# Jaybro/pico_tree

Measured on AMD Instinct MI355X. Metric: Mqueries/sec, knn=1 3D L2, 7.73M-pt tree / 7.20M queries, higher is better.
Workload: dtype f32; 1 GPU; BASELINE configs[1]: cloud L (LiDAR-like room scan), 7733372 tree points / 7200863 queries, knn=1, max_leaf_size=10, sliding midpoint; query_order=generated, reorder=auto, streams=1, parallelism=one batch of 7200863 queries cut into 1 shards, tree replicated, tree_nodes=2395585, tree_depth=32

## Files before the change

### pico_tree_amd/build.py

```python

from __future__ import annotations

import os
import shlex
import subprocess
import sys
from concurrent.futures import ThreadPoolExecutor

_HERE = os.path.dirname(os.path.abspath(__file__))
ROOT = os.path.dirname(_HERE)
CSRC = os.path.join(_HERE, "csrc")
LIB = os.path.join(CSRC, "libptk.so")
OBJ = os.path.join(CSRC, "_obj")
UNITS = ["ptk_family_knn", "ptk_backend", "ptk_family_nd", "ptk_family_radius", "ptk_family_f64", "ptk_family_self",
         "ptk_family_topo", "ptk_family_count"]
SOURCES = [os.path.join(CSRC, u + ".hip") for u in UNITS]

FLAGS = [
    "--offload-arch=gfx950",
    "-O3",
    "-std=c++17",
    "-ffp-contract=off",
    "-fPIC",
    "-Wall",
    "-Wno-unused-result",
    "-Wno-unused-function",
]


def _compile_flags() -> list:
    return FLAGS + os.environ.get("PTK_EXTRA_FLAGS", "").split() + [
        "-I" + os.path.join(ROOT, "include"),
        "-I" + CSRC,
    ]


def _deps(depfile: str) -> list:
    try:
        with open(depfile) as f:
            text = f.read()
    except OSError:
        return []
    text = text.replace("\\\n", " ")
    _, _, rest = text.partition(":")
    return shlex.split(rest)


def _signature(unit: str, flags_line: str) -> str:
    import hashlib

    h = hashlib.sha256(flags_line.replace(os.path.realpath(ROOT), "<root>").replace(ROOT, "<root>").encode())
    deps = sorted(set(os.path.realpath(p) for p in _deps(os.path.join(OBJ, unit + ".d"))))
    root = os.path.realpath(ROOT) + os.sep
    mine = [p for p in deps if p.startswith(root)]
    if not mine:
        return ""
    for p in mine:
        try:
            with open(p, "rb") as f:
                h.update(p[len(root):].encode() + b"\0" + f.read())
        except OSError:
            return ""
    return h.hexdigest()


def _unit_stale(unit: str, flags_line: str) -> bool:
    obj = os.path.join(OBJ, unit + ".o")
    sigfile = os.path.join(OBJ, unit + ".sig")
    if not (os.path.exists(obj) and os.path.exists(sigfile)):
        return True
    with open(sigfile) as f:
        recorded = f.read().strip()
    return recorded == "" or recorded != _signature(unit, flags_line)


def _compile(unit: str, flags: list, flags_line: str, verbose: bool) -> None:
    hipcc = os.environ.get("HIPCC", "/opt/rocm/bin/hipcc")
    obj = os.path.join(OBJ, unit + ".o")
    cmd = [hipcc] + flags + ["-c", "-MD", "-MF", os.path.join(OBJ, unit + ".d"), "-o", obj,
                             os.path.join(CSRC, unit + ".hip")]
    if verbose:
        print(" ".join(cmd), file=sys.stderr)
    subprocess.check_call(cmd)
    with open(os.path.join(OBJ, unit + ".sig"), "w") as f:
        f.write(_signature(unit, flags_line))


def build(force: bool = False, verbose: bool = False, lib: str = LIB) -> str:
    flags = _compile_flags()
    flags_line = " ".join(flags)
    os.makedirs(OBJ, exist_ok=True)
    todo = [u for u in UNITS if force or _unit_stale(u, flags_line)]
    if todo:
        jobs = max(1, min(len(todo), int(os.environ.get("PTK_BUILD_JOBS", os.cpu_count() or 4))))
        with ThreadPoolExecutor(max_workers=jobs) as pool:
            for _ in pool.map(lambda u: _compile(u, flags, flags_line, verbose), todo):
                pass
    objs = [os.path.join(OBJ, u + ".o") for u in UNITS]
    linked = os.path.join(OBJ, os.path.basename(lib) + ".sig")
    want = "\n".join(open(os.path.join(OBJ, u + ".sig")).read() for u in UNITS)
    have = open(linked).read() if os.path.exists(linked) else None
    if todo or not os.path.exists(lib) or have != want:
        hipcc = os.environ.get("HIPCC", "/opt/rocm/bin/hipcc")
        cmd = [hipcc, "--offload-arch=gfx950", "-shared", "-fPIC", "-o", lib] + objs
        if verbose:
            print(" ".join(cmd), file=sys.stderr)
        subprocess.check_call(cmd)
        with open(linked, "w") as f:
            f.write(want)
    return lib


if __name__ == "__main__":
    print(build(force="--force" in sys.argv, verbose=True))
```

### pico_tree_amd/csrc/ptk_backend.hip

```cpp

#include "ptk_families.hpp"
#include "ptk_kernels_lists.hpp"
#include "ptk_piles.hpp"
#include "ptk_build.hpp"
#include "ptk_sort.hpp"
#include "ptk_forest.hpp"
#include "ptk_rows_out.hpp"

namespace {

void axis_bits(const ptk_tree* t, int bits, uint32_t b[3]);

struct CreateClock {
  bool on;
  double* sink;
  std::chrono::steady_clock::time_point t0;
  explicit CreateClock(double* phases = nullptr)
      : on(env_int("PTK_CREATE_TIMING", 0) != 0), sink(phases), t0(std::chrono::steady_clock::now()) {}
  void lap(const char* what, int slot) {
    const auto t1 = std::chrono::steady_clock::now();
    const double ms = std::chrono::duration<double, std::milli>(t1 - t0).count();
    if (sink != nullptr && slot >= 0) sink[slot] += ms;
    if (on) std::fprintf(stderr, "[ptk create] %-28s %8.2f ms\n", what, ms);
    t0 = t1;
// ... 225 lines not shown
  std::mutex lock;
  std::thread threads[kMaxDevices];
  bool started[kMaxDevices] = {};
  void start(int32_t device) {
    if (device == kDeviceNone) return;
    const char* sw = std::getenv("PTK_EAGER_WARMUP");
    if (sw != nullptr && std::atoi(sw) == 0) return;
    int dev = device;
    if (dev < 0 && hipGetDevice(&dev) != hipSuccess) return;
    if (dev < 0 || dev >= kMaxDevices) return;
    std::lock_guard<std::mutex> hold(lock);
    if (started[dev]) return;
    started[dev] = true;
    threads[dev] = std::thread([dev] {
      if (hipSetDevice(dev) != hipSuccess) {
        (void)hipGetLastError();
        return;
      }
      hipLaunchKernelGGL(ptk_warm_kernel, dim3(1), dim3(1), 0, nullptr);
      ptkf::warm_knn();
      ptkf::warm_radius();
      ptkf::warm_nd();
      ptkf::warm_topo();
      ptkf::warm_count();
      ptkf::warm_f64();
      ptkf::warm_self();
      (void)hipDeviceSynchronize();
      (void)hipGetLastError();
    });
  }
  void wait(int32_t device) {
    int dev = device;
    if (dev < 0 && hipGetDevice(&dev) != hipSuccess) return;
    if (dev < 0 || dev >= kMaxDevices) return;
    std::lock_guard<std::mutex> hold(lock);
    if (threads[dev].joinable()) threads[dev].join();
  }
  ~ProcessWarmup() {
    for (auto& th : threads)
      if (th.joinable()) th.join();
  }
};
ProcessWarmup g_warmup;

int finish_create(ptk_tree* t, const float* points, int32_t device, ptk_tree** out) {
  if (t->root_min.empty()) {
    t->root_min.assign(t->dim, std::numeric_limits<float>::max());
    t->root_max.assign(t->dim, std::numeric_limits<float>::lowest());
    for (uint64_t i = 0; i < t->n_points; ++i)
      for (uint32_t d = 0; d < t->dim; ++d) {
        const float v = points[i * t->dim + d];
        t->root_min[d] = std::min(t->root_min[d], v);
        t->root_max[d] = std::max(t->root_max[d], v);
      }
  }
  if (device == kDeviceNone) {
    int rc = analyse(*t);
    if (rc != PTK_OK) {
      delete t;
      return rc;
    }
    t->device = kDeviceNone;
    *out = t;
    return PTK_OK;
  }
  int count = 0;
  if (hipGetDeviceCount(&count) != hipSuccess || count <= 0) {
    delete t;
    return fail(PTK_ERR_DEVICE, "no HIP device is visible");
  }
  int dev = device;
  if (dev < 0 && hipGetDevice(&dev) != hipSuccess) dev = 0;
  if (dev >= count) {
    delete t;
    return fail(PTK_ERR_INVALID, "device %d out of range (%d visible)", dev, count);
  }
  t->device = dev;
  DeviceGuard guard(dev);
  if (!guard.ok) {
    delete t;
    return fail(PTK_ERR_DEVICE, "hipSetDevice(%d) failed", dev);
  }
  {
    hipDeviceProp_t prop;
    if (hipGetDeviceProperties(&prop, dev) == hipSuccess) {
      if (prop.multiProcessorCount > 0) t->cus = prop.multiProcessorCount;
      if (prop.maxSharedMemoryPerMultiProcessor > 0) t->lds_per_cu = prop.maxSharedMemoryPerMultiProcessor;
      const size_t optin = prop.sharedMemPerBlockOptin > 0 ? (size_t)prop.sharedMemPerBlockOptin : (size_t)prop.sharedMemPerBlock;
      if (optin > 0) t->lds_per_block = std::min(optin, t->lds_per_cu);
      t->hbm_bytes = prop.totalGlobalMem;
    } else {
      (void)hipGetLastError();
    }
  }
  int rc = upload(*t, points);
  if (rc != PTK_OK) {
    ptk_tree_destroy(t);
    return rc;
  }
  *out = t;
  return PTK_OK;
}

bool want_reorder(const ptk_tree* t, uint64_t nq) {
  const int mode = t->reorder.load();
  if (mode == PTK_REORDER_ON) return nq > 1;
  if (mode == PTK_REORDER_OFF) return false;
  return nq >= 8192;
}

int morton_bits(uint64_t nq) { return nq < (1ull << 20) ? 16 : 24; }

void axis_bits(const ptk_tree* t, int bits, uint32_t b[3]) {
  b[0] = b[1] = b[2] = 0;
  const uint32_t axes = t->dim < 3 ? t->dim : 3;
  double want[3] = {0, 0, 0};
  const double total = t->axis_splits[0] + t->axis_splits[1] + t->axis_splits[2];
  for (uint32_t a = 0; a < axes; ++a) want[a] = total > 0.0 ? bits * t->axis_splits[a] / total : (double)bits / axes;
  for (int given = 0; given < bits; ++given) {
    int best = -1;
    for (uint32_t a = 0; a < axes; ++a)
      if (b[a] < 15 && (best < 0 || want[a] - b[a] > want[best] - b[best])) best = (int)a;
    if (best < 0) break;
    ++b[best];
  }
}

using MortonSortConfig =
    rocprim::radix_sort_config<rocprim::default_config, rocprim::default_config, rocprim::default_config, 131072>;

size_t sort_tmp_bytes(uint64_t nq, int bits) {
  size_t tmp_bytes = 0;
  uint32_t* k32 = nullptr;
  (void)rocprim::radix_sort_pairs<MortonSortConfig>(nullptr, tmp_bytes, k32, k32, k32, k32, nq, 0, bits,
                                                    (hipStream_t) nullptr);
  return tmp_bytes + 256;
}

uint32_t sort_tile(uint64_t nq) {
  const uint64_t t = ((nq + 4095) / 4096 + 63) & ~(uint64_t)63;
  return (uint32_t)std::max<uint64_t>(t, (uint64_t)512);
}
uint32_t sort_tiles(uint64_t nq) { return (uint32_t)((nq + sort_tile(nq) - 1) / sort_tile(nq)); }
uint32_t sort_stride(uint64_t nq) { return (sort_tiles(nq) + 3u) & ~3u;  }
size_t own_sort_bytes(uint64_t nq) {
  const size_t stride = std::max<size_t>(sort_stride(nq), ((nq + ptk::kSortTile - 1) / ptk::kSortTile + 3) & ~(size_t)3);
  return ((size_t)ptk::kRadixBins * stride + ptk::kRadixBins) * 4 + 2 * nq * sizeof(uint2) + 1024;
}

bool block_sort(uint64_t nq) {
  const int mode = knob_int("sort_block", -1);
  return mode < 0 ? nq >= (3ull << 18) : mode != 0 && nq >= ptk::kSortTile;
}
bool own_sort(uint64_t nq) {
  if (nq >= (1ull << 31)) return false;
  return knob_int("sort", 1) != 0;
}

size_t permutation_scratch_bytes(uint64_t nq) { return 4 * (nq * 4) + sort_tmp_bytes(nq, 30) + own_sort_bytes(nq) + 1024; }

const uint32_t* sample_batch(const ptk_tree* t, const float* d_q, uint64_t nq, hipStream_t s, Scratch& scratch, int bits,
                             const float3& lo3, const float3& inv3, const uint3& b3) {
  if (nq < 8192) return nullptr;
  uint8_t* d_fail = scratch.take<uint8_t>(ptk::kCoherenceWindows);
  uint32_t* state = scratch.sample_state();
  if (d_fail == nullptr || state == nullptr) return nullptr;
  uint32_t lg = 0;
  while ((128ull << lg) <= nq) ++lg;
  const uint32_t max_log2 = (uint32_t)std::min(bits, std::max(bits - (int)lg, 0) + 5);
  hipLaunchKernelGGL(ptk::coherence_sample_kernel, dim3(ptk::kCoherenceWindows), dim3(64), 0, s, d_q, t->dim, nq, lo3, inv3,
                     b3, max_log2, d_fail, state);
  return state + 1;
}

int make_permutation(const ptk_tree* t, const float* d_q, uint64_t nq, hipStream_t s, Scratch& scratch,
                     uint32_t** perm, uint32_t heavy_first = 0, bool may_skip = false) {
  *perm = nullptr;
  if (nq >= (1ull << 32)) return fail(PTK_ERR_UNSUPPORTED, "batches of 2^32 or more queries are not supported");
  Timer timer(t, s);
  const int bits = morton_bits(nq);
  size_t tmp_bytes = sort_tmp_bytes(nq, bits);
  uint32_t* keys = scratch.take<uint32_t>(nq);
  uint32_t* keys_out = scratch.take<uint32_t>(nq);
  uint32_t* ids = scratch.take<uint32_t>(nq);
  uint32_t* ids_out = scratch.take<uint32_t>(nq);
  void* tmp = scratch.take<char>(tmp_bytes);
  if (!keys || !keys_out || !ids || !ids_out || !tmp) return fail(PTK_ERR_NOMEM, "scratch block too small");
  uint32_t b[3];
  axis_bits(t, bits, b);
  float lo[3] = {0, 0, 0}, inv[3] = {0, 0, 0};
  for (uint32_t d = 0; d < t->dim && d < 3; ++d) {
    lo[d] = t->root_min[d];
    const float ext = t->root_max[d] - t->root_min[d];
    inv[d] = ext > 0 ? (float)(1u << b[d]) / ext : 0.0f;
  }
  ptk::CellTable cells{};
  if (heavy_first != 0u && t->cells.occ != nullptr) {
    cells = t->cells;
    cells.key_bits = (uint32_t)bits;
    cells.mode = heavy_first;
  }
  const uint32_t* as_given = may_skip && own_sort(nq)
                                 ? sample_batch(t, d_q, nq, s, scratch, bits, make_float3(lo[0], lo[1], lo[2]),
                                                make_float3(inv[0], inv[1], inv[2]), make_uint3(b[0], b[1], b[2]))
                                 : nullptr;
  scratch.note_verdict(as_given);
  if (own_sort(nq)) {
    const bool blocks = block_sort(nq);
    const uint32_t tile = blocks ? ptk::kSortTile : sort_tile(nq);
    const uint32_t tiles = blocks ? (uint32_t)((nq + tile - 1) / tile) : sort_tiles(nq);
    const uint32_t stride = blocks ? (tiles + 3u) & ~3u : sort_stride(nq);
    uint32_t* hist = scratch.take<uint32_t>((size_t)ptk::kRadixBins * stride);
    uint32_t* totals = scratch.take<uint32_t>(ptk::kRadixBins);
    uint2* pairs_a = scratch.take<uint2>(nq);
    uint2* pairs_b = bits > 16 ? scratch.take<uint2>(nq) : pairs_a;
    if (!hist || !totals || !pairs_a || !pairs_b) return fail(PTK_ERR_NOMEM, "scratch block too small");
    const float3 lo3 = make_float3(lo[0], lo[1], lo[2]), inv3 = make_float3(inv[0], inv[1], inv[2]);
    const uint3 b3 = make_uint3(b[0], b[1], b[2]);
    const int passes = (bits + 7) / 8;
    const size_t smem = ptk::kRadixBins * 4;
    const uint2* in = nullptr;
    for (int p = 0; p < passes; ++p) {
      const uint32_t shift = 8u * (uint32_t)p;
      const bool first = p == 0, last = p + 1 == passes;
      uint2* out = in == pairs_a ? pairs_b : pairs_a;
      if (blocks && first)
        hipLaunchKernelGGL((ptk::radix_block_hist_kernel<true>), dim3(tiles), dim3(ptk::kSortBlock), smem, s, d_q, t->dim,
                           (uint32_t)nq, lo3, inv3, b3, keys, in, shift, stride, hist, cells, as_given);
      else if (blocks)
        hipLaunchKernelGGL((ptk::radix_block_hist_kernel<false>), dim3(tiles), dim3(ptk::kSortBlock), smem, s, d_q, t->dim,
                           (uint32_t)nq, lo3, inv3, b3, keys, in, shift, stride, hist, ptk::CellTable{}, as_given);
      else if (first)
        hipLaunchKernelGGL((ptk::radix_hist_kernel<true>), dim3(tiles), dim3(64), smem, s, d_q, t->dim, (uint32_t)nq, lo3,
                           inv3, b3, keys, in, shift, tile, stride, hist, cells, as_given);
      else
        hipLaunchKernelGGL((ptk::radix_hist_kernel<false>), dim3(tiles), dim3(64), smem, s, d_q, t->dim, (uint32_t)nq, lo3,
                           inv3, b3, keys, in, shift, tile, stride, hist, ptk::CellTable{}, as_given);
      hipLaunchKernelGGL(ptk::radix_scan_kernel, dim3(ptk::kRadixBins), dim3(64), 0, s, hist, tiles, stride, totals);
#define PTK_SCATTER(F, L)                                                                                              \
  if (blocks)                                                                                                          \
    hipLaunchKernelGGL((ptk::radix_block_scatter_kernel<F, L>), dim3(tiles), dim3(ptk::kSortBlock),                    \
                       ptk::kSortScatterLds, s, keys, in, out, ids_out, (uint32_t)nq, shift, stride, hist, totals,     \
                       as_given);                                                                                      \
  else                                                                                                                 \
    hipLaunchKernelGGL((ptk::radix_scatter_kernel<F, L>), dim3(tiles), dim3(64), smem, s, keys, in, out, ids_out,      \
                       (uint32_t)nq, shift, tile, stride, hist, totals, as_given)
      if (first && last) PTK_SCATTER(true, true);
      else if (first) PTK_SCATTER(true, false);
      else if (last) PTK_SCATTER(false, true);
      else PTK_SCATTER(false, false);
#undef PTK_SCATTER
      in = out;
    }
    PTK_HIP(hipGetLastError());
    *perm = ids_out;
    scratch.note_order(1);
    timer.stop(1, 0);
    return PTK_OK;
  }
  {
    const uint32_t blocks = (uint32_t)((nq + ptk::kBlock - 1) / ptk::kBlock);
    hipLaunchKernelGGL(ptk::morton_kernel, dim3(blocks), dim3(ptk::kBlock), 0, s, d_q, t->dim, nq,
                       make_float3(lo[0], lo[1], lo[2]), make_float3(inv[0], inv[1], inv[2]),
                       make_uint3(b[0], b[1], b[2]), keys, ids, cells, (uint64_t)0);
  }
  PTK_HIP(rocprim::radix_sort_pairs<MortonSortConfig>(tmp, tmp_bytes, keys, keys_out, ids, ids_out, nq, 0, bits, s));
  *perm = ids_out;
  scratch.note_order(1);
  timer.stop(1, 0);
  return PTK_OK;
}

int order_batch(const ptk_tree* t, const float* d_q, uint64_t nq, hipStream_t s, Scratch& scratch, size_t extra_bytes,
                uint32_t** perm, uint32_t heavy_first = 0, bool may_skip = false) {
  *perm = nullptr;
  const bool reorder = want_reorder(t, nq);
  const int rc = scratch.reserve(extra_bytes + (reorder ? permutation_scratch_bytes(nq) : 0));
  if (rc != PTK_OK || !reorder) return rc;
  return make_permutation(t, d_q, nq, s, scratch, perm, heavy_first, may_skip);
}

size_t capture_budget_bytes(const ptk_tree* t) {
  const size_t quarter_mb = t->hbm_bytes ? (t->hbm_bytes >> 22) : 16384;
  const int mb = env_int("PTK_RADIUS_CAPTURE_MB", (int)std::min<size_t>(16384, std::max<size_t>(quarter_mb, 64)));
  return mb <= 0 ? 0 : (size_t)mb << 20;
}

bool prepare_capture(const ptk_tree* t, uint64_t nq, Workspace& ws, bool with_heavy = false) {
  const size_t budget = capture_budget_bytes(t);
  if (budget == 0 || nq == 0 || nq >= (1ull << 31)) return false;
  const size_t waves = (size_t)((nq + 63) / 64);
  const size_t chunk_bytes = (size_t)ptk::kLogChunk * sizeof(ptk::Neighbor);
  const size_t flags_at = (size_t)ptk::kCapSubPools * ptk::kCapCounterStride * 4;
  const size_t qids_at = flags_at + ((waves + 255) & ~(size_t)255);
  const size_t lens_at = qids_at + waves * 64 * 4;
  const size_t tables_at = lens_at + waves * 64 * 4;
  const size_t heavy_at = (tables_at + waves * ptk::kListMaxChunks * 4 + 255) & ~(size_t)255;
  const size_t mh = with_heavy ? (size_t)radius_max_handover(nq) : 0, ecap = with_heavy ? (size_t)radius_entry_cap(nq) : 0;
  const size_t heavy_bytes = with_heavy ? 256 + 4 * ((mh * 4 + 255) & ~(size_t)255) + ecap * 8 : 0;
  const size_t head = (heavy_at + heavy_bytes + 4095) & ~(size_t)4095;
  if (head + waves * chunk_bytes > budget) return false;
  const size_t dyn = std::min<size_t>((budget - head - waves * chunk_bytes) / chunk_bytes, waves * 64 * 2);
  const int forced = knob_int("radius_capture_chunks", -1);
  size_t sub_cap = forced >= 0 ? (size_t)forced : dyn / ptk::kCapSubPools;
  const size_t max_chunks = ((1ull << 32) - 1) / ptk::kLogChunk;
  if (waves >= max_chunks) return false;
  if (waves + sub_cap * ptk::kCapSubPools > max_chunks) sub_cap = (max_chunks - waves) / ptk::kCapSubPools;
  const size_t bytes = head + (waves + sub_cap * ptk::kCapSubPools) * chunk_bytes;
  if (bytes > ws.cap_capacity) {
    drain_workspace(ws);
    if (ws.cap_base) (void)hipFree(ws.cap_base);
    ws.cap_base = nullptr;
    ws.cap_capacity = 0;
    ws.cap_valid = false;
    size_t free_b = 0, total_b = 0;
    if (hipMemGetInfo(&free_b, &total_b) != hipSuccess || bytes > free_b / 2) return false;
    if (hipMalloc((void**)&ws.cap_base, bytes) != hipSuccess) {
      (void)hipGetLastError();
      ws.cap_base = nullptr;
      return false;
    }
    ws.cap_capacity = bytes;
  }
  ws.cap.counters = reinterpret_cast<uint32_t*>(ws.cap_base);
  ws.cap.captured = reinterpret_cast<uint8_t*>(ws.cap_base + flags_at);
  ws.cap.qids = reinterpret_cast<uint32_t*>(ws.cap_base + qids_at);
  ws.cap.lens = reinterpret_cast<uint32_t*>(ws.cap_base + lens_at);
  ws.cap.tables = reinterpret_cast<uint32_t*>(ws.cap_base + tables_at);
  ws.cap.chunks = reinterpret_cast<ptk::Neighbor*>(ws.cap_base + head);
  ws.cap.n_static = (uint32_t)waves;
  ws.cap.sub_cap = (uint32_t)sub_cap;
  ws.cap_heavy = ptk::RadiusHeavy{};
  if (with_heavy) {
    const size_t row = (mh * 4 + 255) & ~(size_t)255;
    char* p = ws.cap_base + heavy_at;
    ws.cap_heavy.meta = reinterpret_cast<uint32_t*>(p);
    ws.cap_heavy.rows = reinterpret_cast<uint32_t*>(p + 256);
    ws.cap_heavy.own = reinterpret_cast<uint32_t*>(p + 256 + row);
    ws.cap_heavy.run_at = reinterpret_cast<uint32_t*>(p + 256 + 2 * row);
    ws.cap_heavy.run_n = reinterpret_cast<uint32_t*>(p + 256 + 3 * row);
    ws.cap_heavy.entries = reinterpret_cast<unsigned long long*>(p + 256 + 4 * row);
    ws.cap_heavy.max_heavy = (uint32_t)mh;
    ws.cap_heavy.entry_cap = (uint32_t)std::min<size_t>(ecap, 0xFFFFFFFFu);
  }
  return true;
}

ptk::TierSpec phase2_tiers(uint32_t cap) {
  ptk::TierSpec t{};
  if (cap == 0) {
    t.permille[0] = 60;
    t.lanes[0] = 4;
  }
  return t;
}

size_t class_sort_tmp_bytes(uint64_t nq) {
  size_t tmp_bytes = 0;
  ptk::ContKey* k16 = nullptr;
  uint32_t* v32 = nullptr;
  (void)rocprim::radix_sort_pairs(nullptr, tmp_bytes, k16, k16, v32, v32, nq, 0, 16, (hipStream_t) nullptr);
  return tmp_bytes + 256;
}

uint64_t max_handover(uint64_t nq) { return std::max<uint64_t>(nq / 32, std::min<uint64_t>(nq, 16384)); }

struct ClassPlan {
  uint32_t ntiles, stride, seg, segs, per, chunks;
};
ClassPlan class_plan(uint64_t nq) {
  ClassPlan p;
  p.ntiles = (uint32_t)((nq + 63) / 64);
  p.stride = (p.ntiles + 3u) & ~3u;
// ... 2099 lines not shown
```

### pico_tree_amd/csrc/ptk_sort.hpp

```cpp

#pragma once

#include <hip/hip_runtime.h>
#include <stdint.h>

#include "ptk_kernels.hpp"

namespace ptk {

constexpr uint32_t kRadixBins = 256;

__device__ __forceinline__ uint64_t same_digit_lanes(uint32_t digit, bool valid) {
  uint64_t peers = __ballot(valid);
#pragma unroll
  for (uint32_t b = 0; b < 8; ++b) {
    const bool bit = ((digit >> b) & 1u) != 0u;
    const uint64_t m = __ballot(bit);
    peers &= bit ? m : ~m;
  }
  return peers;
}

__device__ __forceinline__ uint32_t wave_inclusive_sum(uint32_t v, uint32_t lane) {
#pragma unroll
// ... 148 lines not shown
        const uint32_t dst = p + (uint32_t)__popcll(peers & below);
        if (LAST) vals_out[dst] = val[u];
        else pairs_out[dst] = make_uint2(key[u], val[u]);
        if ((peers >> lane) == 1ull) pos[digit] = p + (uint32_t)__popcll(peers);
      }
    }
  }
}

constexpr uint32_t kSortBlock = 512, kSortItems = 8, kSortTile = kSortBlock * kSortItems;
constexpr uint32_t sort_scatter_lds(uint32_t block, uint32_t items) {
  return ((block / 64u) * kRadixBins + 2u * kRadixBins + 32u) * 4u + block * items * 8u;
}
constexpr uint32_t kSortScatterLds = sort_scatter_lds(kSortBlock, kSortItems);

__device__ __forceinline__ uint32_t block_exclusive_sum(uint32_t v, uint32_t t, PTK_LDS uint32_t* tmp) {
  const uint32_t lane = t & 63u, w = t >> 6;
  const uint32_t incl = wave_inclusive_sum(v, lane);
  if (lane == 63u && w < 4u) tmp[w] = incl;
  __syncthreads();
  uint32_t before = 0;
#pragma unroll
  for (uint32_t j = 0; j < 3; ++j) before += j < w ? tmp[j] : 0u;
  __syncthreads();
  return before + incl - v;
}

template <bool FROM_QUERIES, uint32_t BLOCK = kSortBlock, uint32_t ITEMS = kSortItems>
__global__ __launch_bounds__(BLOCK) void radix_block_hist_kernel(
    const float* __restrict__ queries, uint32_t dim, uint32_t nq, float3 lo, float3 inv, uint3 bits,
    uint32_t* __restrict__ keys, const uint2* __restrict__ pairs, uint32_t shift, uint32_t stride,
    uint32_t* __restrict__ hist, CellTable cells = CellTable{}, const uint32_t* __restrict__ as_given = nullptr) {
  if (as_given != nullptr && *as_given != 0u) return;
  typedef PTK_LDS uint32_t LdsU32;
  LdsU32* cnt = (LdsU32*)ptk_smem;
  const uint32_t t = threadIdx.x;
  if (t < kRadixBins) cnt[t] = 0u;
  __syncthreads();
  const uint32_t base = blockIdx.x * (BLOCK * ITEMS);
  uint32_t key[ITEMS];
  bool valid[ITEMS];
  if (FROM_QUERIES) {
    float x[ITEMS], y[ITEMS], z[ITEMS];
#pragma unroll
    for (uint32_t j = 0; j < ITEMS; ++j) {
      const uint32_t i = base + j * BLOCK + t;
      valid[j] = i < nq;
      load_query(queries, dim, valid[j] ? i : nq - 1u, x[j], y[j], z[j]);
    }
#pragma unroll
    for (uint32_t j = 0; j < ITEMS; ++j) {
      key[j] = order_key(x[j], y[j], z[j], lo, inv, bits, cells);
      if (valid[j]) keys[base + j * BLOCK + t] = key[j];
    }
  } else {
#pragma unroll
    for (uint32_t j = 0; j < ITEMS; ++j) {
      const uint32_t i = base + j * BLOCK + t;
      valid[j] = i < nq;
      key[j] = valid[j] ? pairs[i].x : 0u;
    }
  }
#pragma unroll
  for (uint32_t j = 0; j < ITEMS; ++j) {
    if (valid[j]) lds_add_u32(&cnt[(key[j] >> shift) & 255u], 1u);
  }
  __syncthreads();
  if (t < kRadixBins) hist[t * stride + blockIdx.x] = cnt[t];
}

template <bool FIRST, bool LAST, uint32_t BLOCK = kSortBlock, uint32_t ITEMS = kSortItems>
__global__ __launch_bounds__(BLOCK) void radix_block_scatter_kernel(
    const uint32_t* __restrict__ keys_in, const uint2* __restrict__ pairs_in, uint2* __restrict__ pairs_out,
    uint32_t* __restrict__ vals_out, uint32_t n, uint32_t shift, uint32_t stride, const uint32_t* __restrict__ hist,
    const uint32_t* __restrict__ totals, const uint32_t* __restrict__ as_given = nullptr) {
  if (as_given != nullptr && *as_given != 0u) return;
  constexpr uint32_t WAVES = BLOCK / 64u, TILE = BLOCK * ITEMS;
  static_assert(BLOCK >= kRadixBins && BLOCK % 64u == 0u, "a thread per digit");
  typedef PTK_LDS uint32_t LdsU32;
  LdsU32* wave_cnt = (LdsU32*)ptk_smem;
  LdsU32* lbase = wave_cnt + WAVES * kRadixBins;
  LdsU32* gbase = lbase + kRadixBins;
  LdsU32* tmp = gbase + kRadixBins;
  LdsWord* buf = (LdsWord*)(tmp + 32);
  const uint32_t t = threadIdx.x, lane = t & 63u, w = t >> 6;
  const uint32_t base = blockIdx.x * TILE;
  for (uint32_t j = t; j < WAVES * kRadixBins; j += BLOCK) wave_cnt[j] = 0u;
  uint32_t key[ITEMS], val[ITEMS], rank[ITEMS];
  bool valid[ITEMS];
#pragma unroll
  for (uint32_t r = 0; r < ITEMS; ++r) {
    const uint32_t i = base + w * (ITEMS * 64u) + r * 64u + lane;
    valid[r] = i < n;
    if (FIRST) {
      key[r] = valid[r] ? keys_in[i] : 0u;
      val[r] = i;
    } else {
      const uint2 p = valid[r] ? pairs_in[i] : make_uint2(0u, 0u);
      key[r] = p.x;
      val[r] = p.y;
    }
  }
  __syncthreads();
  const uint64_t below = (1ull << lane) - 1ull;
#pragma unroll
  for (uint32_t r = 0; r < ITEMS; ++r) {
    const uint32_t digit = (key[r] >> shift) & 255u;
    const uint64_t peers = same_digit_lanes(digit, valid[r]);
    const uint32_t before = wave_cnt[w * kRadixBins + (valid[r] ? digit : 0u)];
    rank[r] = before + (uint32_t)__popcll(peers & below);
    if (valid[r] && (peers >> lane) == 1ull) wave_cnt[w * kRadixBins + digit] = before + (uint32_t)__popcll(peers);
  }
  __syncthreads();
  {
    uint32_t sum = 0;
    if (t < kRadixBins) {
#pragma unroll
      for (uint32_t j = 0; j < WAVES; ++j) {
        const uint32_t c = wave_cnt[j * kRadixBins + t];
        wave_cnt[j * kRadixBins + t] = sum;
        sum += c;
      }
    }
    const uint32_t in_tile = block_exclusive_sum(t < kRadixBins ? sum : 0u, t, tmp);
    const uint32_t in_all = block_exclusive_sum(t < kRadixBins ? totals[t] : 0u, t, tmp + 8);
    if (t < kRadixBins) {
      lbase[t] = in_tile;
      gbase[t] = in_all + hist[t * stride + blockIdx.x];
    }
  }
  __syncthreads();
#pragma unroll
  for (uint32_t r = 0; r < ITEMS; ++r) {
    if (valid[r]) {
      const uint32_t digit = (key[r] >> shift) & 255u;
      buf[lbase[digit] + wave_cnt[w * kRadixBins + digit] + rank[r]] = (unsigned long long)key[r] | ((unsigned long long)val[r] << 32);
    }
  }
  __syncthreads();
  const uint32_t held = n - base < TILE ? n - base : TILE;
#pragma unroll
  for (uint32_t j = 0; j < ITEMS; ++j) {
    const uint32_t at = j * BLOCK + t;
    if (at < held) {
      const unsigned long long kv = buf[at];
      const uint32_t digit = ((uint32_t)kv >> shift) & 255u;
      const uint32_t dst = gbase[digit] + (at - lbase[digit]);
      if (LAST) vals_out[dst] = (uint32_t)(kv >> 32);
      else pairs_out[dst] = make_uint2((uint32_t)kv, (uint32_t)(kv >> 32));
    }
  }
}

}
```

Baseline: 4919 Mqueries/s.

## Add narrow radix sort path with byte digit histograms and packed pairs

Adds a new query-ordering radix sort path, on by default for large batches. The scatter pass writes the next pass's 8-bit digit into a byte array, so later histogram passes read one byte per item instead of the whole key/value pair. It also optionally packs the key remainder and row index into one 32-bit word for the final pass, and stages 3D query rows through LDS with float4 loads when building the first-pass keys. This cuts memory traffic in the sort preprocessing, at the cost of extra digit writes and more kernel variants. Separately, the build script gains an early exit when the linked library is already current.

```diff
diff --git a/pico_tree_amd/build.py b/pico_tree_amd/build.py
--- a/pico_tree_amd/build.py
+++ b/pico_tree_amd/build.py
@@ -74,6 +74,20 @@
     return recorded == "" or recorded != _signature(unit, flags_line)
 
 
+def _library_current(lib: str, flags_line: str) -> bool:
+    linked = os.path.join(OBJ, os.path.basename(lib) + ".sig")
+    if not (os.path.exists(lib) and os.path.exists(linked)):
+        return False
+    sigs = []
+    for unit in UNITS:
+        sig = _signature(unit, flags_line)
+        if sig == "":
+            return False
+        sigs.append(sig)
+    with open(linked) as f:
+        return f.read() == "\n".join(sigs)
+
+
 def _compile(unit: str, flags: list, flags_line: str, verbose: bool) -> None:
     hipcc = os.environ.get("HIPCC", "/opt/rocm/bin/hipcc")
     obj = os.path.join(OBJ, unit + ".o")
@@ -90,6 +104,8 @@
     flags = _compile_flags()
     flags_line = " ".join(flags)
     os.makedirs(OBJ, exist_ok=True)
+    if not force and _library_current(lib, flags_line):
+        return lib
     todo = [u for u in UNITS if force or _unit_stale(u, flags_line)]
     if todo:
         jobs = max(1, min(len(todo), int(os.environ.get("PTK_BUILD_JOBS", os.cpu_count() or 4))))
diff --git a/pico_tree_amd/csrc/ptk_backend.hip b/pico_tree_amd/csrc/ptk_backend.hip
--- a/pico_tree_amd/csrc/ptk_backend.hip
+++ b/pico_tree_amd/csrc/ptk_backend.hip
@@ -401,6 +401,11 @@
   const int mode = knob_int("sort_block", -1);
   return mode < 0 ? nq >= (3ull << 18) : mode != 0 && nq >= ptk::kSortTile;
 }
+uint32_t narrow_sort(uint64_t nq) {
+  if (!block_sort(nq)) return 0u;
+  const int mode = knob_int("sort_narrow", knob_int("sort_block", -1) < 0 ? 7 : 0);
+  return mode > 0 ? (uint32_t)mode | 1u : 0u;
+}
 bool own_sort(uint64_t nq) {
   if (nq >= (1ull << 31)) return false;
   return knob_int("sort", 1) != 0;
@@ -468,6 +473,53 @@
     const uint3 b3 = make_uint3(b[0], b[1], b[2]);
     const int passes = (bits + 7) / 8;
     const size_t smem = ptk::kRadixBins * 4;
+    if (const uint32_t narrow = narrow_sort(nq)) {
+      uint8_t* digits = reinterpret_cast<uint8_t*>(keys_out);
+      const bool staged = (narrow & 4u) != 0u && t->dim == 3 && (reinterpret_cast<uintptr_t>(d_q) & 15u) == 0u;
+      const bool pack = (narrow & 2u) != 0u && nq <= (1ull << ptk::kPackedRowBits);
+      const void* from = keys;
+      uint32_t from_kind = ptk::kItemKeys;
+      for (int p = 0; p < passes; ++p) {
+        const uint32_t shift = 8u * (uint32_t)p;
+        const bool last = p + 1 == passes;
+        void* to = last ? (void*)ids_out : from == pairs_a ? (void*)pairs_b : (void*)pairs_a;
+        const uint32_t to_kind = last ? ptk::kItemRows : pack && bits - 8 * (p + 1) <= 8 ? ptk::kItemPacked : ptk::kItemPairs;
+        if (p > 0)
+          hipLaunchKernelGGL((ptk::radix_digit_hist_kernel<>), dim3(tiles), dim3(ptk::kSortBlock), smem, s, digits,
+                             (uint32_t)nq, stride, hist, as_given);
+        else if (staged)
+          hipLaunchKernelGGL((ptk::radix_key_hist_kernel<true>), dim3(tiles), dim3(ptk::kSortBlock), ptk::kSortKeyStagedLds,
+                             s, d_q, t->dim, (uint32_t)nq, lo3, inv3, b3, keys, shift, stride, hist, cells, as_given);
+        else
+          hipLaunchKernelGGL((ptk::radix_key_hist_kernel<false>), dim3(tiles), dim3(ptk::kSortBlock), ptk::kSortKeyLds, s,
+                             d_q, t->dim, (uint32_t)nq, lo3, inv3, b3, keys, shift, stride, hist, cells, as_given);
+        hipLaunchKernelGGL(ptk::radix_scan_kernel, dim3(ptk::kRadixBins), dim3(64), 0, s, hist, tiles, stride, totals);
+#define PTK_NARROW(IN, OUT)                                                                                            \
+  case (IN) * 4u + (OUT):                                                                                              \
+    hipLaunchKernelGGL((ptk::radix_narrow_scatter_kernel<IN, OUT>), dim3(tiles), dim3(ptk::kSortBlock),                \
+                       ptk::kSortScatterLds, s, from, to, last ? nullptr : digits, (uint32_t)nq, shift, stride, hist,  \
+                       totals, as_given);                                                                              \
+    break
+        switch (from_kind * 4u + to_kind) {
+          PTK_NARROW(ptk::kItemKeys, ptk::kItemPairs);
+          PTK_NARROW(ptk::kItemKeys, ptk::kItemPacked);
+          PTK_NARROW(ptk::kItemKeys, ptk::kItemRows);
+          PTK_NARROW(ptk::kItemPairs, ptk::kItemPairs);
+          PTK_NARROW(ptk::kItemPairs, ptk::kItemPacked);
+          PTK_NARROW(ptk::kItemPairs, ptk::kItemRows);
+          PTK_NARROW(ptk::kItemPacked, ptk::kItemRows);
+          default: return fail(PTK_ERR_UNSUPPORTED, "batch order: no scatter for this pair of item layouts");
+        }
+#undef PTK_NARROW
+        from = to;
+        from_kind = to_kind;
+      }
+      PTK_HIP(hipGetLastError());
+      *perm = ids_out;
+      scratch.note_order(1);
+      timer.stop(1, 0);
+      return PTK_OK;
+    }
     const uint2* in = nullptr;
     for (int p = 0; p < passes; ++p) {
       const uint32_t shift = 8u * (uint32_t)p;
diff --git a/pico_tree_amd/csrc/ptk_sort.hpp b/pico_tree_amd/csrc/ptk_sort.hpp
--- a/pico_tree_amd/csrc/ptk_sort.hpp
+++ b/pico_tree_amd/csrc/ptk_sort.hpp
@@ -324,4 +324,240 @@
   }
 }
 
-}
+constexpr uint32_t kItemKeys = 0;
+constexpr uint32_t kItemPairs = 1;
+constexpr uint32_t kItemPacked = 2;
+constexpr uint32_t kItemRows = 3;
+constexpr uint32_t kPackedRowBits = 24;
+constexpr uint32_t kSortKeyLds = kRadixBins * 4u;
+constexpr uint32_t kSortKeyStagedLds = kSortKeyLds + kSortTile * 3u * 4u;
+
+template <uint32_t N>
+__device__ __forceinline__ void morton_keys(const float (&x)[N], const float (&y)[N], const float (&z)[N], float3 lo,
+                                            float3 inv, uint3 bits, uint32_t (&key)[N]) {
+  uint32_t cx[N], cy[N], cz[N];
+#pragma unroll
+  for (uint32_t j = 0; j < N; ++j) {
+    cx[j] = (uint32_t)fminf(fmaxf((x[j] - lo.x) * inv.x, 0.0f), (float)((1u << bits.x) - 1u));
+    cy[j] = (uint32_t)fminf(fmaxf((y[j] - lo.y) * inv.y, 0.0f), (float)((1u << bits.y) - 1u));
+    cz[j] = (uint32_t)fminf(fmaxf((z[j] - lo.z) * inv.z, 0.0f), (float)((1u << bits.z) - 1u));
+    key[j] = 0u;
+  }
+  const uint32_t top = bits.x > bits.y ? (bits.x > bits.z ? bits.x : bits.z) : (bits.y > bits.z ? bits.y : bits.z);
+  for (uint32_t level = top; level-- > 0;) {
+    if (bits.z > level) {
+#pragma unroll
+      for (uint32_t j = 0; j < N; ++j) key[j] = (key[j] << 1) | ((cz[j] >> level) & 1u);
+    }
+    if (bits.y > level) {
+#pragma unroll
+      for (uint32_t j = 0; j < N; ++j) key[j] = (key[j] << 1) | ((cy[j] >> level) & 1u);
+    }
+    if (bits.x > level) {
+#pragma unroll
+      for (uint32_t j = 0; j < N; ++j) key[j] = (key[j] << 1) | ((cx[j] >> level) & 1u);
+    }
+  }
+}
+template <uint32_t N>
+__device__ __forceinline__ void order_keys(const float (&x)[N], const float (&y)[N], const float (&z)[N], float3 lo,
+                                           float3 inv, uint3 bits, const CellTable& cells, uint32_t (&key)[N]) {
+  morton_keys<N>(x, y, z, lo, inv, bits, key);
+  if (cells.occ == nullptr) return;
+  uint32_t cell[N];
+  morton_keys<N>(x, y, z, lo, cells.inv, cells.bits, cell);
+#pragma unroll
+  for (uint32_t j = 0; j < N; ++j) {
+    const uint32_t v = cells.occ[cell[j]];
+    if (cells.mode == kCellsEmptyFirst) {
+      key[j] = ((v != 0u ? 1u : 0u) << (cells.key_bits - 1u)) | (key[j] >> 1);
+    } else {
+      const uint32_t cls = v >= 12u ? 0u : (v >= 10u ? 1u : (v >= 8u ? 2u : 3u));
+      key[j] = (cls << (cells.key_bits - 2u)) | (key[j] >> 2);
+    }
+  }
+}
+
+template <bool STAGED, uint32_t BLOCK = kSortBlock, uint32_t ITEMS = kSortItems>
+__global__ __launch_bounds__(BLOCK) void radix_key_hist_kernel(
+    const float* __restrict__ queries, uint32_t dim, uint32_t nq, float3 lo, float3 inv, uint3 bits,
+    uint32_t* __restrict__ keys, uint32_t shift, uint32_t stride, uint32_t* __restrict__ hist, CellTable cells = CellTable{},
+    const uint32_t* __restrict__ as_given = nullptr) {
+  if (as_given != nullptr && *as_given != 0u) return;
+  constexpr uint32_t TILE = BLOCK * ITEMS;
+  static_assert((TILE * 3u) % 4u == 0u && (TILE * 12u) % 16u == 0u, "a tile of rows is a whole number of 16-byte pieces");
+  typedef PTK_LDS uint32_t LdsU32;
+  typedef PTK_LDS float LdsF32;
+  LdsU32* cnt = (LdsU32*)ptk_smem;
+  const uint32_t t = threadIdx.x;
+  if (t < kRadixBins) cnt[t] = 0u;
+  const uint32_t base = blockIdx.x * TILE;
+  float x[ITEMS], y[ITEMS], z[ITEMS];
+  bool valid[ITEMS];
+  if (STAGED) {
+    LdsF32* rows = (LdsF32*)(ptk_smem + kSortKeyLds);
+    const uint32_t held = nq - base < TILE ? nq - base : TILE;
+    const uint32_t floats = held * 3u;
+    const float* src = queries + (uint64_t)base * 3u;
+    constexpr uint32_t PIECES = TILE * 3u / 4u;
+#pragma unroll
+    for (uint32_t j = 0; j < (PIECES + BLOCK - 1u) / BLOCK; ++j) {
+      const uint32_t piece = j * BLOCK + t, f = piece * 4u;
+      if (piece < PIECES && f + 4u <= floats) {
+        const float4 v = reinterpret_cast<const float4*>(src)[piece];
+        rows[f] = v.x;
+        rows[f + 1u] = v.y;
+        rows[f + 2u] = v.z;
+        rows[f + 3u] = v.w;
+      } else if (piece < PIECES && f < floats) {
+        for (uint32_t c = f; c < floats; ++c) rows[c] = src[c];
+      }
+    }
+    __syncthreads();
+#pragma unroll
+    for (uint32_t j = 0; j < ITEMS; ++j) {
+      const uint32_t r = j * BLOCK + t;
+      valid[j] = r < held;
+      x[j] = valid[j] ? rows[3u * r] : 0.0f;
+      y[j] = valid[j] ? rows[3u * r + 1u] : 0.0f;
+      z[j] = valid[j] ? rows[3u * r + 2u] : 0.0f;
+    }
+  } else {
+#pragma unroll
+    for (uint32_t j = 0; j < ITEMS; ++j) {
+      const uint32_t i = base + j * BLOCK + t;
+      valid[j] = i < nq;
+      load_query(queries, dim, valid[j] ? i : nq - 1u, x[j], y[j], z[j]);
+    }
+    __syncthreads();
+  }
+  uint32_t key[ITEMS];
+  order_keys<ITEMS>(x, y, z, lo, inv, bits, cells, key);
+#pragma unroll
+  for (uint32_t j = 0; j < ITEMS; ++j) {
+    if (valid[j]) {
+      keys[base + j * BLOCK + t] = key[j];
+      lds_add_u32(&cnt[(key[j] >> shift) & 255u], 1u);
+    }
+  }
+  __syncthreads();
+  if (t < kRadixBins) hist[t * stride + blockIdx.x] = cnt[t];
+}
+
+template <uint32_t BLOCK = kSortBlock, uint32_t ITEMS = kSortItems>
+__global__ __launch_bounds__(BLOCK) void radix_digit_hist_kernel(const uint8_t* __restrict__ digits, uint32_t n,
+                                                                 uint32_t stride, uint32_t* __restrict__ hist,
+                                                                 const uint32_t* __restrict__ as_given = nullptr) {
+  if (as_given != nullptr && *as_given != 0u) return;
+  static_assert(ITEMS == 8u, "a thread's digits are one 8-byte load");
+  typedef PTK_LDS uint32_t LdsU32;
+  LdsU32* cnt = (LdsU32*)ptk_smem;
+  const uint32_t t = threadIdx.x;
+  if (t < kRadixBins) cnt[t] = 0u;
+  __syncthreads();
+  const uint32_t first = blockIdx.x * (BLOCK * ITEMS) + t * ITEMS;
+  if (first < n) {
+    const uint2 d = reinterpret_cast<const uint2*>(digits)[first / ITEMS];
+    const uint32_t have = n - first < ITEMS ? n - first : ITEMS;
+#pragma unroll
+    for (uint32_t j = 0; j < ITEMS; ++j) {
+      const uint32_t digit = ((j < 4u ? d.x : d.y) >> (8u * (j & 3u))) & 255u;
+      if (j < have) lds_add_u32(&cnt[digit], 1u);
+    }
+  }
+  __syncthreads();
+  if (t < kRadixBins) hist[t * stride + blockIdx.x] = cnt[t];
+}
+
+template <uint32_t IN, uint32_t OUT, uint32_t BLOCK = kSortBlock, uint32_t ITEMS = kSortItems>
+__global__ __launch_bounds__(BLOCK) void radix_narrow_scatter_kernel(
+    const void* __restrict__ items_in, void* __restrict__ items_out, uint8_t* __restrict__ digits_out, uint32_t n,
+    uint32_t shift, uint32_t stride, const uint32_t* __restrict__ hist, const uint32_t* __restrict__ totals,
+    const uint32_t* __restrict__ as_given = nullptr) {
+  if (as_given != nullptr && *as_given != 0u) return;
+  constexpr uint32_t WAVES = BLOCK / 64u, TILE = BLOCK * ITEMS;
+  static_assert(BLOCK >= kRadixBins && BLOCK % 64u == 0u, "a thread per digit");
+  static_assert(IN != kItemRows && OUT != kItemKeys, "rows only leave, keys only enter");
+  typedef PTK_LDS uint32_t LdsU32;
+  LdsU32* wave_cnt = (LdsU32*)ptk_smem;
+  LdsU32* lbase = wave_cnt + WAVES * kRadixBins;
+  LdsU32* gbase = lbase + kRadixBins;
+  LdsU32* tmp = gbase + kRadixBins;
+  LdsWord* buf = (LdsWord*)(tmp + 32);
+  const uint32_t t = threadIdx.x, lane = t & 63u, w = t >> 6;
+  const uint32_t base = blockIdx.x * TILE;
+  for (uint32_t j = t; j < WAVES * kRadixBins; j += BLOCK) wave_cnt[j] = 0u;
+  uint32_t key[ITEMS], val[ITEMS], rank[ITEMS];
+  bool valid[ITEMS];
+#pragma unroll
+  for (uint32_t r = 0; r < ITEMS; ++r) {
+    const uint32_t i = base + w * (ITEMS * 64u) + r * 64u + lane;
+    valid[r] = i < n;
+    if (IN == kItemKeys) {
+      key[r] = valid[r] ? static_cast<const uint32_t*>(items_in)[i] : 0u;
+      val[r] = i;
+    } else if (IN == kItemPairs) {
+      const uint2 p = valid[r] ? static_cast<const uint2*>(items_in)[i] : make_uint2(0u, 0u);
+      key[r] = p.x;
+      val[r] = p.y;
+    } else {
+      const uint32_t p = valid[r] ? static_cast<const uint32_t*>(items_in)[i] : 0u;
+      key[r] = (p >> kPackedRowBits) << shift;
+      val[r] = p & ((1u << kPackedRowBits) - 1u);
+    }
+  }
+  __syncthreads();
+  const uint64_t below = (1ull << lane) - 1ull;
+#pragma unroll
+  for (uint32_t r = 0; r < ITEMS; ++r) {
+    const uint32_t digit = (key[r] >> shift) & 255u;
+    const uint64_t peers = same_digit_lanes(digit, valid[r]);
+    const uint32_t before = wave_cnt[w * kRadixBins + (valid[r] ? digit : 0u)];
+    rank[r] = before + (uint32_t)__popcll(peers & below);
+    if (valid[r] && (peers >> lane) == 1ull) wave_cnt[w * kRadixBins + digit] = before + (uint32_t)__popcll(peers);
+  }
+  __syncthreads();
+  {
+    uint32_t sum = 0;
+    if (t < kRadixBins) {
+#pragma unroll
+      for (uint32_t j = 0; j < WAVES; ++j) {
+        const uint32_t c = wave_cnt[j * kRadixBins + t];
+        wave_cnt[j * kRadixBins + t] = sum;
+        sum += c;
+      }
+    }
+    const uint32_t in_tile = block_exclusive_sum(t < kRadixBins ? sum : 0u, t, tmp);
+    const uint32_t in_all = block_exclusive_sum(t < kRadixBins ? totals[t] : 0u, t, tmp + 8);
+    if (t < kRadixBins) {
+      lbase[t] = in_tile;
+      gbase[t] = in_all + hist[t * stride + blockIdx.x];
+    }
+  }
+  __syncthreads();
+#pragma unroll
+  for (uint32_t r = 0; r < ITEMS; ++r) {
+    if (valid[r]) {
+      const uint32_t digit = (key[r] >> shift) & 255u;
+      buf[lbase[digit] + wave_cnt[w * kRadixBins + digit] + rank[r]] = (unsigned long long)key[r] | ((unsigned long long)val[r] << 32);
+    }
+  }
+  __syncthreads();
+  const uint32_t held = n - base < TILE ? n - base : TILE;
+#pragma unroll
+  for (uint32_t j = 0; j < ITEMS; ++j) {
+    const uint32_t at = j * BLOCK + t;
+    if (at < held) {
+      const unsigned long long kv = buf[at];
+      const uint32_t k = (uint32_t)kv, v = (uint32_t)(kv >> 32);
+      const uint32_t digit = (k >> shift) & 255u;
+      const uint32_t dst = gbase[digit] + (at - lbase[digit]);
+      if (OUT == kItemRows) static_cast<uint32_t*>(items_out)[dst] = v;
+      else if (OUT == kItemPacked) static_cast<uint32_t*>(items_out)[dst] = ((k >> (shift + 8u)) << kPackedRowBits) | v;
+      else static_cast<uint2*>(items_out)[dst] = make_uint2(k, v);
+      if (OUT != kItemRows && digits_out != nullptr) digits_out[dst] = (uint8_t)((k >> (shift + 8u)) & 255u);
+    }
+  }
+}
+
+}
```

Result: faster. 4977 Mqueries/s (median of 6 runs) (+1.2%).
